# neherlab/pangraph

Measured on AMD Instinct MI355X. Metric: aligned Gbp/s in `pangraph build` (bases handed to the aligner per second, all merges, all self-merge rounds), higher is better.
Workload: dtype u8

## Files before the change

dev/strips_probe.py:

```python
import sys, os, time, faulthandler
ROOT = os.path.dirname(os.path.dirname(os.path.abspath(__file__))); os.chdir(ROOT); sys.path.insert(0, ROOT); sys.path.insert(0, ROOT + '/tests')
faulthandler.dump_traceback_later(240, exit=True)
import numpy as np
import stagebind as sb
from pangraph_amd.mm2ffi import Mm2Lib
from pangraph_amd.synth import random_seq, mutate
gpu = Mm2Lib('pangraph_amd/libpgalign.so')
rng = np.random.default_rng(7)
def job(L, fl, kind):
    t = random_seq(rng, L)
    q = random_seq(rng, L) if kind == "junk" else mutate(rng, t, snp=0.01, indel=0.001)
    if kind == "half": q = np.concatenate([q[:L // 2], random_seq(rng, L // 2)])
    return (sb.nt4(q.tobytes().decode()), sb.nt4(t.tobytes().decode()), 150001, 200, -1, fl)
for L in (10000, 4000, 2048):
    for kind in ("junk", "half", "related"):
        for fl, name in ((0x08, "approx"), (0, "exact")):
            jobs = [job(L, fl, kind)]
            sb.product_extd2(gpu.dll, jobs, 1, 9, 1, 16, 2, 41, 1)
            best = 1e9
            for rep in range(3):
                t0 = time.time(); r = sb.product_extd2(gpu.dll, jobs, 1, 9, 1, 16, 2, 41, 1); best = min(best, time.time() - t0)
            print(f"L={L} {kind:8s} {name:6s}: {best*1e3:7.2f} ms wall; zdropped={r[0]['zdropped']} n_cigar={len(r[0]['cigar'])} score={r[0]['score']}", flush=True)
```

pangraph_amd/csrc/pga_dp.h:

```cpp
#pragma once
#include "pga_common.h"

namespace pga {

struct DpJob {
	uint64_t t_off;
	uint64_t q_off;
	int32_t qlen_full;
	int32_t qs;
	int32_t qlen, tlen;
	int32_t w, zdrop, end_bonus, flag;
	uint8_t q_rev;
	uint8_t seq_rev;
	uint8_t pad[2];
};

struct DpRes {
	int32_t max, max_q, max_t, mqe, mqe_t, mte, mte_q, score;
	int32_t zdropped, reach_end, n_cigar, pad;
	uint64_t cigar_off;
};

#define PGA_JOB_LL 0x8000
#define PGA_LL_MAX_LEN 10240
// ... 5 lines not shown
#include "pga_ksw_shared.h"

namespace pga {

struct LbStop { int32_t on, r_lo, r_hi, tail; };
__host__ __device__ inline int32_t lb_gap(int q, int e, int q2, int e2, int L) { const int a = q + e * L, b = q2 + e2 * L; return a < b ? a : b; }
__host__ __device__ inline LbStop lb_stop_of(int qlen, int tlen, int w, int flag, int q, int e, int q2, int e2, int sc_mch, int sc_mis, int sc_N, int lb_mode)
{
	LbStop S; S.on = 0; S.r_lo = S.r_hi = S.tail = 0;
	if (lb_mode == 1 || (flag & (EZ_APPROX_MAX | PGA_JOB_LL)) || tlen > 64 || tlen < 1 || w < 64 || qlen < w + 2 * tlen) return S;
	if (sc_mch < 0 || sc_mis > sc_mch || sc_N > sc_mch || q < 0 || e < 0 || q2 < 0 || e2 < 0) return S;
	S.on = 1; S.r_lo = 2 * tlen; S.r_hi = w + 30;
	const int qe1 = q + e < q2 + e2 ? q + e : q2 + e2;
	S.tail = tlen > 16 ? sc_mch * tlen - lb_gap(q, e, q2, e2, w + 32 - 2 * tlen) + (sc_mch + qe1) * (2 * tlen - 32) : (int32_t)0x80000000;
	return S;
}
__host__ __device__ inline bool lb_final(const LbStop &S, int r, int tlen, int q, int e, int q2, int e2, int sc_mch, int m)
{
	return S.on && r >= S.r_lo && r <= S.r_hi && sc_mch * tlen - lb_gap(q, e, q2, e2, r + 3 - 2 * tlen) <= m && S.tail <= m;
}

int dp_lb_mode();
void dp_routes_take(int64_t by_class[14], int64_t handed_back[2]);
size_t dp_slab_bytes(int qlen, int tlen, int w);
void dp_run(PkBases d_bases, const std::vector<DpJob> &jobs, const DpParams &P, std::vector<DpRes> &res, PinVec<uint32_t> &cigars, hipStream_t st, Timers *tm = nullptr);

void launch_extd2_fast(int C, unsigned n_waves, const DpJob *jobs, uint32_t n_jobs, PkBases bases, const DpParams &P, uint32_t *counter, uint8_t *slab, size_t slab_bytes,
                       DpRes *res, uint32_t *pool, unsigned long long *cursor, unsigned long long pool_cap, hipStream_t st);

size_t wide_lds_bytes(int r_cap, int seq_cap, bool exact);
void launch_extd2_wide(unsigned n_blocks, int n_threads, int r_cap, int seq_cap, bool exact, const DpJob *jobs, uint32_t n_jobs, PkBases bases, const DpParams &P, uint32_t *counter, uint8_t *slab, size_t slab_bytes,
                       DpRes *res, uint32_t *pool, unsigned long long *cursor, unsigned long long pool_cap, hipStream_t st);

size_t ll_lds_bytes(int t_cap);
size_t ll_multi_scratch_bytes();
int ll_groups(uint32_t n_jobs, int t_max);
void launch_ll_multi(int G, int t_cap, const DpJob *jobs, uint32_t n_jobs, PkBases bases, const DpParams &P, unsigned long long *scratch, DpRes *res, hipStream_t st);
void launch_ll_i16(unsigned n_blocks, int t_cap, const DpJob *jobs, uint32_t n_jobs, PkBases bases, const DpParams &P, uint32_t *counter,
                   unsigned long long *rowkey, size_t rowkey_stride, DpRes *res, hipStream_t st);

size_t band_slab_bytes(int max_diag);
void launch_gapfill_band(unsigned n_waves, const DpJob *jobs, uint32_t n_jobs, PkBases bases, const DpParams &P, uint32_t *counter, uint8_t *slab, size_t slab_bytes,
                         DpRes *res, uint32_t *pool, unsigned long long *cursor, unsigned long long pool_cap, hipStream_t st);

bool strips_eligible(const DpJob &j, const DpParams &P);
size_t strips_slab_bytes(const DpJob &j);
int strips_count(const DpJob &j);
size_t strips_bnd_words(const DpJob &j);
void launch_approx_strips(unsigned n_blocks, const DpJob *jobs, const uint32_t *blk_job, const uint32_t *blk_strip, PkBases bases, const DpParams &P, uint8_t *slab, const uint64_t *slab_off,
                          uint32_t *bnd, const uint64_t *bnd_off, uint32_t *done_ctr, DpRes *res, uint32_t *pool, unsigned long long *cursor, unsigned long long pool_cap, hipStream_t st);

bool wstrips_on();
bool wstrips_eligible(const DpJob &j, const DpParams &P);
int wstrips_count(const DpJob &j);
size_t wstrips_bnd_words(const DpJob &j);
void launch_wstrips(unsigned n_blocks, const DpJob *jobs, const uint32_t *blk_job, const uint32_t *blk_strip, PkBases bases, const DpParams &P, uint8_t *slab, const uint64_t *slab_off,
                    unsigned long long *bnd, const uint64_t *bnd_off, uint32_t *done_ctr, DpRes *res, uint32_t *pool, unsigned long long *cursor, unsigned long long pool_cap, hipStream_t st);
int bstrips_mode();
int bstrips_max_problems();
int bstrips_long_diagonals();
bool bstrips_eligible(const DpJob &j, const DpParams &P);
size_t bstrips_slab_bytes(const DpJob &j);
size_t bstrips_words(const DpJob &j);
uint32_t bstrips_table(const DpJob &j, std::vector<uint32_t> &tab, size_t *words);
void launch_bstrips(unsigned n_blocks, const DpJob *jobs, const uint32_t *blk_job, PkBases bases, const DpParams &P, uint8_t *slab, const uint64_t *slab_off,
                    unsigned long long *bnd, const uint64_t *bnd_off, const uint32_t *tab, const uint64_t *tab_off, DpRes *res, uint32_t *pool, unsigned long long *cursor,
                    unsigned long long pool_cap, hipStream_t st);
bool pipe_eligible(const DpJob &j);
int pipe_mode();
size_t pipe_cig_bytes(int q_cap, int t_cap);
size_t pipe_chunk_bytes();
int pipe_max_chunks();
void launch_ext_pipe(unsigned n_blocks, int q_cap, int t_cap, const DpJob *jobs, uint32_t n_jobs, PkBases bases, const DpParams &P, uint32_t *counter, uint8_t *slab, uint32_t n_chunks,
                     DpRes *res, uint32_t *pool, unsigned long long *cursor, unsigned long long pool_cap, hipStream_t st);
bool lanes_eligible(const DpJob &j, int nt);
size_t lanes_cig_bytes(int q_cap, int t_cap);
size_t lanes_chunk_bytes(int nt);
void launch_extd2_lanes(int nt, unsigned n_blocks, int q_cap, int t_cap, const DpJob *jobs, uint32_t n_jobs, PkBases bases, const DpParams &P, uint32_t *counter, uint8_t *slab, uint32_t n_chunks,
                        DpRes *res, uint32_t *pool, unsigned long long *cursor, unsigned long long pool_cap, hipStream_t st);

}
```

pangraph_amd/csrc/pga_ksw.hip:

```cpp
#include "pga_common.h"
#include "pga_ksw_shared.h"
#include <atomic>
#include <chrono>
#include <mutex>
#include <thread>
#include <array>
#include <cstdio>
#include <cstring>

namespace pga {

#define LDS_T 2048

__global__ __launch_bounds__(64)
void k_extd2(const DpJob *__restrict__ jobs, uint32_t n_jobs, PkBases bases, DpParams P,
             uint32_t *__restrict__ job_counter, uint8_t *__restrict__ slab_all, size_t slab_bytes,
             DpRes *__restrict__ res, uint32_t *__restrict__ cigar_pool, unsigned long long *__restrict__ pool_cursor, unsigned long long pool_cap)
{
	__shared__ int8_t s_rows[7 * LDS_T];
	__shared__ int32_t s_H[LDS_T];
	__shared__ uint32_t s_job;
	const int lane = threadIdx.x;
	uint8_t *slab = slab_all + (size_t)blockIdx.x * slab_bytes;

// ... 578 lines not shown
		lane_need[lane_of_class[c]] = std::max(lane_need[lane_of_class[c]], n_waves * slab_max[c]);
	}
	LaneLease lanes(dev_id, lane_need);
	struct DrainUncollected {
		std::vector<Launch> &L; int dev;
		~DrainUncollected() { for (Launch &X : L) if (X.si >= 0) { (void)sync_stream(X.cs); dp_stream_done(dp_stream_pool(dev), X.si, X.est); X.si = -1; } }
	} drain_uncollected{L, dev_id};
	hipStream_t *lane_stream = lanes.set->stream;
	DBuf<uint8_t> *lane_slab = lanes.set->slab;
	for (int l = 0; l < DP_NLANE; ++l) if (lane_need[l] > lane_slab[l].cap) {
		ArenaScope own(lanes.set->arena);
		g_slab_total -= lane_slab[l].cap; lane_slab[l].alloc(lane_need[l]); g_slab_total += lane_slab[l].cap;
	}
	int lane_si[DP_NLANE] = {-1, -1, -1, -1, -1, -1, -1, -1, -1};
	static const int launch_order[DP_NCLASS] = {13, 12, 9, 11, 7, 6, 5, 4, 3, 10, 2, 8, 1, 0};
	for (int oi = 0; oi < DP_NCLASS; ++oi) {
		const int c = launch_order[oi];
		if (cls[c].empty()) continue;
		std::vector<uint32_t> &ids = cls[c];
		if ((c >= 2 && c != 8) || ids.size() < 100000)
			std::stable_sort(ids.begin(), ids.end(), [&](uint32_t a, uint32_t b) { return (size_t)jobs[a].qlen * jobs[a].tlen > (size_t)jobs[b].qlen * jobs[b].tlen; });
		L.emplace_back();
		Launch &X = L.back();
		X.c = c; X.ids = &ids;
		PinVec<DpJob> &jb = X.jb; jb.resize(ids.size());
		host_parallel(ids.size(), [&](size_t lo, size_t hi) { for (size_t i = lo; i < hi; ++i) jb[i] = jobs[ids[i]]; });
		static const size_t zc_max = getenv("PGA_DP_ZEROCOPY_MAX") ? (size_t)atol(getenv("PGA_DP_ZEROCOPY_MAX")) : 2048;
		X.zc = ids.size() <= zc_max;
		if (X.zc) { X.hr.resize(ids.size()); X.jobs_p = jb.data(); X.res_p = X.hr.data(); }
		else { X.d_jobs.alloc(ids.size()); X.d_r.alloc(ids.size()); X.jobs_p = X.d_jobs.p; X.res_p = X.d_r.p; }
		if (c == 9) { X.d_cnt.alloc(ids.size()); X.cnt_p = X.d_cnt.p; } else X.cnt_p = reinterpret_cast<uint32_t*>(d_cursor.p + 1 + c);
		X.n_waves = waves_of[c];
		uint8_t *slab_p = lane_slab[lane_of_class[c]].p;
		static const bool serial = getenv("PGA_DP_SERIAL") != nullptr;
		hipStream_t cs;
		if (dp_shared_streams()) {
			static const double base_ms[DP_NCLASS] = {1.5, 2.0, 4.0, 6.0, 10.0, 10.0, 10.0, 10.0, 0.5, 12.0, 5.0, 4.0, 2.0, 3.0};
			double est = base_ms[c] * std::max(1.0, (double)ids.size() / (c <= 1 || c == 8 ? 20000.0 : c == 10 || c == 11 || c == 13 ? 512.0 : 64.0));
			DpStreamPool &SP = dp_stream_pool(dev_id);
			int &lsi = lane_si[lane_of_class[c]];
			if (lsi < 0) lsi = dp_stream_pick(SP, est);
			else { std::lock_guard<std::mutex> lk(SP.mu); SP.load[(size_t)lsi] += est; ++SP.pending[(size_t)lsi]; }
			X.si = lsi; X.est = est; cs = SP.st[(size_t)X.si];
		} else cs = lane_stream[serial ? 0 : lane_of_class[c]];
		X.cs = cs;
		if (!X.zc) PGA_HIP(hipMemcpyAsync(X.d_jobs.p, jb.data(), jb.size() * sizeof(DpJob), hipMemcpyHostToDevice, cs));
		if (c == 9) PGA_HIP(hipMemsetAsync(X.d_cnt.p, 0, sizeof(uint32_t) * X.d_cnt.n, cs));
		PGA_HIP(hipEventCreate(&X.e0)); PGA_HIP(hipEventCreate(&X.e1));
		PGA_HIP(hipEventRecord(X.e0, cs));
		if (c == 9) {
			std::vector<uint32_t> &bj = X.h_bj, &bs = X.h_bs; std::vector<uint64_t> &so = X.h_so, &bo = X.h_bo; so.assign(ids.size(), 0); bo.assign(ids.size(), 0);
			uint64_t s_acc = 0, b_acc = 0;
			const bool ws = wstrips_on();
			for (size_t i = 0; i < ids.size(); ++i) {
				const DpJob &j = jobs[ids[i]];
				so[i] = s_acc; s_acc += need[ids[i]];
				bo[i] = b_acc; b_acc += ws ? wstrips_bnd_words(j) : strips_bnd_words(j);
				for (int k2 = 0; k2 < (ws ? wstrips_count(j) : strips_count(j)); ++k2) { bj.push_back((uint32_t)i); bs.push_back((uint32_t)k2); }
			}
			X.d_blk_job.upload(bj, cs); X.d_blk_strip.upload(bs, cs); X.d_slab_off.upload(so, cs); X.d_bnd_off.upload(bo, cs);
			X.d_bnd.alloc(((size_t)b_acc + 1) * (ws ? 2 : 1)); X.d_bnd.zero(cs);
			if (ws) launch_wstrips((unsigned)bj.size(), X.jobs_p, X.d_blk_job.p, X.d_blk_strip.p, d_bases, P, slab_p, X.d_slab_off.p, (unsigned long long*)X.d_bnd.p, X.d_bnd_off.p, X.cnt_p, X.res_p, d_pool.p, d_cursor.p, cig_total, cs);
			else
			launch_approx_strips((unsigned)bj.size(), X.jobs_p, X.d_blk_job.p, X.d_blk_strip.p, d_bases, P, slab_p, X.d_slab_off.p, X.d_bnd.p, X.d_bnd_off.p, X.cnt_p, X.res_p, d_pool.p, d_cursor.p, cig_total, cs);
		} else if (c == 12) {
			std::vector<uint32_t> &bj = X.h_bj, &tab = X.h_tab; std::vector<uint64_t> &so = X.h_so, &bo = X.h_bo, &to = X.h_to; so.assign(ids.size(), 0); bo.assign(ids.size(), 0); to.assign(ids.size(), 0);
			uint64_t s_acc = 0, b_acc = 0;
			for (size_t i = 0; i < ids.size(); ++i) {
				const DpJob &j = jobs[ids[i]];
				so[i] = s_acc; s_acc += need[ids[i]];
				to[i] = tab.size();
				size_t words = 0;
				const uint32_t pool_waves = bstrips_table(j, tab, &words);
				bo[i] = b_acc; b_acc += words;
				for (uint32_t k2 = 0; k2 < pool_waves; ++k2) bj.push_back((uint32_t)i);
			}
			X.d_blk_job.upload(bj, cs); X.d_slab_off.upload(so, cs); X.d_bnd_off.upload(bo, cs); X.d_tab.upload(tab, cs); X.d_tab_off.upload(to, cs);
			X.d_bnd.alloc(((size_t)b_acc + 1) * 2); X.d_bnd.zero(cs);
			X.n_waves = bj.size();
			launch_bstrips((unsigned)bj.size(), X.jobs_p, X.d_blk_job.p, d_bases, P, slab_p, X.d_slab_off.p, (unsigned long long*)X.d_bnd.p, X.d_bnd_off.p, X.d_tab.p, X.d_tab_off.p,
			               X.res_p, d_pool.p, d_cursor.p, cig_total, cs);
		} else if (c == 8) launch_gapfill_band((unsigned)X.n_waves, X.jobs_p, (uint32_t)ids.size(), d_bases, P, X.cnt_p, slab_p, slab_max[c], X.res_p, d_pool.p, d_cursor.p, cig_total, cs);
		else if (c == 6) {
			int t_cap = 16, t_max = 1;
			for (uint32_t id : ids) { t_cap = std::max(t_cap, std::max((jobs[id].tlen + 15) / 16 * 16, (jobs[id].qlen + 15) / 16 * 16)); t_max = std::max(t_max, jobs[id].tlen); }
			const int G = ll_groups((uint32_t)ids.size(), t_max);
			if (G > 1 && ids.size() * ll_multi_scratch_bytes() <= X.n_waves * slab_max[c])
				launch_ll_multi(G, t_cap, X.jobs_p, (uint32_t)ids.size(), d_bases, P, (unsigned long long*)slab_p, X.res_p, cs);
			else
				launch_ll_i16((unsigned)X.n_waves, t_cap, X.jobs_p, (uint32_t)ids.size(), d_bases, P, X.cnt_p, (unsigned long long*)slab_p, slab_max[c] / 8, X.res_p, cs);
		} else if (c <= 1) launch_extd2_fast(c == 0 ? 4 : 8, (unsigned)X.n_waves, X.jobs_p, (uint32_t)ids.size(), d_bases, P, X.cnt_p, slab_p, slab_max[c], X.res_p, d_pool.p, d_cursor.p, cig_total, cs);
		else if (c == 13) {
			int q_cap = 16, t_cap = 16;
			for (uint32_t id : ids) q_cap = std::max(q_cap, jobs[id].qlen), t_cap = std::max(t_cap, jobs[id].tlen);
			launch_ext_pipe((unsigned)X.n_waves, q_cap, t_cap, X.jobs_p, (uint32_t)ids.size(), d_bases, P, X.cnt_p, slab_p, pipe_pool_chunks, X.res_p, d_pool.p, d_cursor.p, cig_total, cs);
		} else if (c == 10 || c == 11) {
			int q_cap = 16, t_cap = 16;
			for (uint32_t id : ids) q_cap = std::max(q_cap, jobs[id].qlen), t_cap = std::max(t_cap, jobs[id].tlen);
			launch_extd2_lanes(c == 11 ? 64 : 256, (unsigned)X.n_waves, q_cap, t_cap, X.jobs_p, (uint32_t)ids.size(), d_bases, P, X.cnt_p, slab_p, lanes_pool_chunks[c - 10], X.res_p, d_pool.p, d_cursor.p, cig_total, cs);
		} else if (c <= 4 || c == 7) {
			int r_cap = 0, seq_cap = 0; bool exact = false;
			for (uint32_t id : ids) { r_cap = std::max(r_cap, wide_ring(jobs[id])); seq_cap = std::max(seq_cap, wide_seqcap(jobs[id])); exact |= !(jobs[id].flag & EZ_APPROX_MAX); }
			if (wide_lds_bytes(r_cap, seq_cap, exact) > WIDE_LDS_MAX) seq_cap = 0;
			static const int c2_seq = getenv("PGA_C2_SEQ") ? atoi(getenv("PGA_C2_SEQ")) : 0;
			if (c == 2 && ids.size() > 1536 && !c2_seq) seq_cap = 0;
			int nt = 256;
			if (c == 4 || c == 7 || ids.size() <= 512) nt = r_cap >= 3000 ? 1024 : r_cap >= 1200 ? 512 : 256;
			if (getenv("PGA_WIDE_NT")) nt = atoi(getenv("PGA_WIDE_NT"));
			else if (c == 3) nt = 512;
			X.nt = nt;
			launch_extd2_wide((unsigned)X.n_waves, nt, r_cap, seq_cap, exact, X.jobs_p, (uint32_t)ids.size(), d_bases, P, X.cnt_p, slab_p, slab_max[c], X.res_p, d_pool.p, d_cursor.p, cig_total, cs);
		} else hipLaunchKernelGGL(k_extd2, dim3((unsigned)X.n_waves), dim3(64), 0, cs, X.jobs_p, (uint32_t)ids.size(), d_bases, P, X.cnt_p, slab_p, slab_max[c],
		                        X.res_p, d_pool.p, d_cursor.p, cig_total);
		PGA_HIP(hipGetLastError());
		PGA_HIP(hipEventRecord(X.e1, cs));
// ... 82 lines not shown
```

pangraph_amd/csrc/pga_ksw_wstrips.hip:

```cpp
#include "pga_common.h"
#include "pga_ksw_shared.h"
#include <cstring>

namespace pga {

#define WS_W 64

__device__ __forceinline__ int ws_sx8(uint32_t v, int sh) { return __builtin_amdgcn_sbfe((int)v, sh, 8); }
__device__ __forceinline__ unsigned long long ws_readlane64(unsigned long long v, int l)
{
	const uint32_t lo = (uint32_t)__builtin_amdgcn_readlane((int)(uint32_t)v, l), hi = (uint32_t)__builtin_amdgcn_readlane((int)(uint32_t)(v >> 32), l);
	return (unsigned long long)hi << 32 | lo;
}

template <bool EXACT>
__device__ __forceinline__ void wstrip_body(const DpJob &J, const uint32_t jl, const uint32_t k, uint8_t *s_win, PkBases bases, const DpParams &P,
               uint8_t *__restrict__ slab_all, const uint64_t *__restrict__ slab_off, unsigned long long *__restrict__ bnd_all, const uint64_t *__restrict__ bnd_off,
               uint32_t *__restrict__ done_ctr, DpRes *__restrict__ res, uint32_t *__restrict__ cigar_pool, unsigned long long *__restrict__ pool_cursor, unsigned long long pool_cap)
{
	const int lane = threadIdx.x;
	const SeqView SV(bases, J);
	const int qlen = J.qlen, tlen = J.tlen;
	const GapCosts G(P);
	const int q = G.q, e = G.e, q2 = G.q2, e2 = G.e2, qe = G.qe, qe2 = G.qe2;
	const int sc_mch = P.sc_mch, sc_mis = P.sc_mis, sc_N = G.sc_N;
	const int qe_h = G.qe_h;
	const int n_strips = (tlen + WS_W - 1) / WS_W;
	const size_t Ld = (size_t)(qlen + tlen);
	const int c0 = (int)k * WS_W, c1 = c0 + WS_W < tlen ? c0 + WS_W : tlen;
	int n_col = qlen < tlen ? qlen : tlen;
	n_col = ((n_col + 15) / 16 + 1) * 16;
	uint8_t *pmat = slab_all + slab_off[jl];
	uint32_t *cig_tmp = (uint32_t*)(pmat + (((size_t)(qlen + tlen - 1) * n_col + 15) & ~(size_t)15));
	unsigned long long *bnd = bnd_all + bnd_off[jl];
	const unsigned long long *bnd_in = k > 0 ? bnd + (size_t)(k - 1) * Ld : nullptr;
	unsigned long long *bnd_out = (int)k + 1 < n_strips ? bnd + (size_t)k * Ld : nullptr;
	int32_t *hen_arr = (int32_t*)(bnd + (size_t)(n_strips > 1 ? n_strips - 1 : 0) * Ld), *hst_arr = hen_arr + Ld;
	const int t = c0 + lane;
	const bool has_col = t < tlen;
	const int tb = SV.target_any(t);
	const int u_first = G.first_row(t);
	int U = u_first, Y = -q - e, Y2 = -q2 - e2, H = KSW_NEG_INF;
	uint32_t PK = ((uint32_t)(-q - e) & 0xffu) | ((uint32_t)(-q - e) & 0xffu) << 8 | ((uint32_t)(-q2 - e2) & 0xffu) << 16;
	int qb = 0;
	const int r_first = c0, r_last = c1 - 1 + qlen - 1;
	const int d_last = c0 + qlen - 2;
	const bool out_strip = bnd_out != nullptr;
	unsigned long long outw = 0;
	uint32_t *s_key = (uint32_t*)s_win;
	unsigned long long *best_arr = (unsigned long long*)(hst_arr + Ld);
	int jq = -lane - 1;
	uint8_t *prow = pmat + (size_t)r_first * n_col;
	{ int st0, en0; diag_range(r_first, qlen, tlen, st0, en0); prow -= st0 / 16 * 16; }
	for (int it0 = 0; r_first + it0 <= r_last; it0 += 64) {
		const int qwin = SV.query(it0 + lane);
		unsigned long long inw = 0;
		{
			const int d = r_first - 1 + it0 + lane;
			if (bnd_in) {
				if (d >= c0 - 1 && d <= d_last)
					for (;;) { inw = __hip_atomic_load(&bnd_in[d], __ATOMIC_RELAXED, __HIP_MEMORY_SCOPE_AGENT); if (inw >> 31 & 1ULL) break; __builtin_amdgcn_s_sleep(2); }
			} else {
				const int rr = d + 1, v1 = G.first_row(rr);
				inw = (unsigned long long)(uint32_t)KSW_NEG_INF << 32 | (((uint32_t)(-q - e) & 0xffu) | ((uint32_t)v1 & 0xffu) << 8 | ((uint32_t)(-q2 - e2) & 0xffu) << 16);
			}
		}
		const int i_end = __builtin_amdgcn_readfirstlane(r_last - (r_first + it0) + 1 < 64 ? r_last - (r_first + it0) + 1 : 64);
		for (int i = 0; i < i_end; ++i) {
			const int r = r_first + it0 + i;
			qb = wave_shr1(qb, __builtin_amdgcn_readlane(qwin, i));
			++jq;
			const bool active = has_col && (unsigned)jq < (unsigned)qlen;
			const uint32_t lw = (uint32_t)wave_shr1((int)PK, __builtin_amdgcn_readlane((int)(uint32_t)inw, i));
			const int xl = ws_sx8(lw, 0), vl = ws_sx8(lw, 8), x2l = ws_sx8(lw, 16);
			int Hl = 0;
			if (EXACT) Hl = wave_shr1(H, __builtin_amdgcn_readlane((int)(uint32_t)(inw >> 32), i));
			int z = tb == qb ? sc_mch : sc_mis;
			z = ((tb | qb) & 4) ? sc_N : z;
			int a = xl + vl, b = Y + U, a2 = x2l + vl, b2 = Y2 + U;
			int d = a > z ? 1 : 0; z = a > z ? a : z;
			d = b > z ? 2 : d; z = b > z ? b : z;
			d = a2 > z ? 3 : d; z = a2 > z ? a2 : z;
			d = b2 > z ? 4 : d; z = b2 > z ? b2 : z;
			z = z < sc_mch ? z : sc_mch;
			const int un = z - vl, vn = z - U;
			int tmp = z - q; a -= tmp; b -= tmp;
			tmp = z - q2; a2 -= tmp; b2 -= tmp;
			d |= a > 0 ? 0x08 : 0; d |= b > 0 ? 0x10 : 0; d |= a2 > 0 ? 0x20 : 0; d |= b2 > 0 ? 0x40 : 0;
			const int xn = (a > 0 ? a : 0) - qe, yn = (b > 0 ? b : 0) - qe, x2n = (a2 > 0 ? a2 : 0) - qe2, y2n = (b2 > 0 ? b2 : 0) - qe2;
			if (active) {
				U = un; Y = yn; Y2 = y2n;
				PK = ((uint32_t)xn & 0xffu) | ((uint32_t)vn & 0xffu) << 8 | ((uint32_t)x2n & 0xffu) << 16;
				prow[(uint32_t)t] = (uint8_t)d;
			}
			if (EXACT) {
				int st0, en0;
				diag_range(r, qlen, tlen, st0, en0);
				uint32_t key = 0;
				if (active) {
					const int en1 = st0 + (en0 - st0) / 4 * 4;
					int h; uint32_t field;
					if (t == en0) { h = r == 0 ? vn - qe_h : en0 > 0 ? Hl + un : H + vn; field = 8u; hen_arr[r] = h; }
					else { h = H + vn; field = 7u - (t < en1 ? (uint32_t)((t - st0) & 3) : 4u); }
					H = h;
					if (t == st0 && r - st0 == qlen - 1) hst_arr[r] = h;
					const int hc = h < -32768 ? -32768 : h > 32767 ? 32767 : h;
					key = ((uint32_t)(hc + 32768) << 16) | field << 12 | (uint32_t)(63 - lane);
				}
				s_key[i * 65 + lane] = key;
			}
			if (out_strip) {
				const uint32_t w63 = (uint32_t)__builtin_amdgcn_readlane((int)PK, 63);
				const bool on63 = (unsigned)(r - (c0 + 63)) < (unsigned)qlen;
				unsigned long long w = on63 ? (0x80000000ULL | w63) : 0ULL;
				if (EXACT) w |= (unsigned long long)(uint32_t)__builtin_amdgcn_readlane(H, 63) << 32;
				if (lane == i) outw = on63 ? w : 0ULL;
			}
			prow += n_col;
			if (r + 2 - qlen > 0 && ((r + 2 - qlen) & 15) == 0) prow -= 16;
		}
		if (out_strip && outw) { __hip_atomic_store(&bnd_out[r_first + it0 + lane], outw, __ATOMIC_RELAXED, __HIP_MEMORY_SCOPE_AGENT); }
		outw = 0;
		if (EXACT) {
			__builtin_amdgcn_fence(__ATOMIC_SEQ_CST, "wavefront");
			if (lane < i_end) {
				uint32_t kb = 0;
#pragma unroll 16
				for (int l = 0; l < 64; ++l) { const uint32_t o = s_key[lane * 65 + l]; kb = o > kb ? o : kb; }
				const unsigned long long comb = (unsigned long long)(kb >> 12) << 20 | (unsigned long long)(4095 - (int)k) << 8 | (unsigned long long)(kb & 255u);
				if (kb) atomicMax(&best_arr[r_first + it0 + lane], comb);
			}
			__builtin_amdgcn_fence(__ATOMIC_SEQ_CST, "wavefront");
		}
	}
	__threadfence();
	uint32_t last = 0;
	if (lane == 0) last = atomicAdd(&done_ctr[jl], 1u);
	last = (uint32_t)__builtin_amdgcn_readfirstlane((int)last);
	if (last + 1 != (uint32_t)n_strips) return;
	__threadfence();
	int bi = tlen - 1, bj = qlen - 1;
	int ez_max = 0, ez_max_t = -1, ez_max_q = -1, ez_mqe = KSW_NEG_INF, ez_mqe_t = -1, ez_mte = KSW_NEG_INF, ez_mte_q = -1, zdropped = 0;
	if (EXACT) {
		const int n_diag = qlen + tlen - 1, zdrop = J.zdrop;
		int sat = 0;
		for (int r0 = 0; r0 < n_diag && !zdropped; r0 += 64) {
			const int r = r0 + lane;
			unsigned long long best = 0; int hen = KSW_NEG_INF, hst = KSW_NEG_INF;
			if (r < n_diag) {
				int st0, en0; diag_range(r, qlen, tlen, st0, en0);
				best = best_arr[r];
				hen = hen_arr[r];
				if (r - st0 == qlen - 1) hst = hst_arr[r];
			}
			const uint32_t h16 = (uint32_t)(best >> 24) & 0xffffu;
			const int mH_l = (int)h16 - 32768, mt_l = (4095 - (int)((best >> 8) & 4095)) * WS_W + (63 - (int)(best & 255));
			const int sat_l = r < n_diag && (h16 == 0 || h16 == 65535u) ? 1 : 0;
			const int lim = n_diag - r0 < 64 ? n_diag - r0 : 64;
			for (int ii = 0; ii < lim; ++ii) {
				const int rr = r0 + ii;
				const int mH = __builtin_amdgcn_readlane(mH_l, ii), mt = __builtin_amdgcn_readlane(mt_l, ii);
				const int he = __builtin_amdgcn_readlane(hen, ii), hs = __builtin_amdgcn_readlane(hst, ii);
				sat |= __builtin_amdgcn_readlane(sat_l, ii);
				int st0, en0; diag_range(rr, qlen, tlen, st0, en0);
				if (en0 == tlen - 1 && he > ez_mte) ez_mte = he, ez_mte_q = rr - en0;
				if (rr - st0 == qlen - 1 && hs > ez_mqe) ez_mqe = hs, ez_mqe_t = st0;
				if (mH > ez_max) ez_max = mH, ez_max_t = mt, ez_max_q = rr - mt;
				else if (mt >= ez_max_t && rr - mt >= ez_max_q) {
					const int tl = mt - ez_max_t, ql = (rr - mt) - ez_max_q, l = tl > ql ? tl - ql : ql - tl;
					if (zdrop >= 0 && ez_max - mH > zdrop + l * e2) { zdropped = 1; break; }
				}
			}
		}
		if (sat) {
			if (lane == 0) { DpRes R; memset(&R, 0, sizeof(R)); R.n_cigar = -9; res[jl] = R; }
			return;
		}
		if (zdropped) bi = ez_max_t, bj = ez_max_q;
	}
	long long guard = 0;
	const int n_cigar = backtrack_windowed<BT_WIN, false>(lane, bi, bj, s_win, cig_tmp, guard, 4000000,
		[&](int r, int &st0, int &en0) { diag_range(r, qlen, tlen, st0, en0); },
		[&](int r, int col) -> uint8_t {
			int st0, en0; diag_range(r, qlen, tlen, st0, en0);
			return st0 <= en0 && col >= st0 && col <= en0 ? pmat[(size_t)r * n_col + (col - st0 / 16 * 16)] : (uint8_t)0;
		});
	__builtin_amdgcn_fence(__ATOMIC_SEQ_CST, "workgroup");
	int score = KSW_NEG_INF;
	if (n_cigar > 0 && !zdropped) {
		int ti = tlen, qj = qlen; score = qe - qe_h;
		for (int c = 0; c < n_cigar; ++c) {
			const uint32_t op = cig_tmp[c] & 0xf; const int len = (int)(cig_tmp[c] >> 4);
			if (op == 0) {
				ti -= len, qj -= len;
				int n_mis = 0, n_amb = 0;
				for (int b = 0; b < len; b += 64) {
					const int l = b + lane;
					bool mis = false, amb = false;
					if (l < len) { const int x = SV.target_any(ti + l), y = SV.query(qj + l); amb = ((x | y) & 4) != 0; mis = !amb && x != y; }
					n_mis += __popcll(__ballot(mis)); n_amb += __popcll(__ballot(amb));
				}
				score += sc_mch * (len - n_mis - n_amb) + sc_mis * n_mis + sc_N * n_amb;
			} else {
				const int g1 = q + len * e, g2 = q2 + len * e2;
				score -= g1 < g2 ? g1 : g2;
				if (op == 1) qj -= len; else ti -= len;
			}
		}
	}
	DpRes R = ez_record(ez_max, ez_max_q, ez_max_t, ez_mqe, ez_mqe_t, ez_mte, ez_mte_q, score, zdropped, 0);
	R.n_cigar = n_cigar, R.pad = qlen + tlen - 1;
	cigar_commit<false, true>(lane, n_cigar, false, cig_tmp, cigar_pool, pool_cursor, pool_cap, R, &res[jl]);
}

__global__ __launch_bounds__(64)
void k_wstrips(const DpJob *__restrict__ jobs, const uint32_t *__restrict__ blk_job, const uint32_t *__restrict__ blk_strip, PkBases bases, DpParams P,
               uint8_t *__restrict__ slab_all, const uint64_t *__restrict__ slab_off, unsigned long long *__restrict__ bnd_all, const uint64_t *__restrict__ bnd_off,
               uint32_t *__restrict__ done_ctr, DpRes *__restrict__ res, uint32_t *__restrict__ cigar_pool, unsigned long long *__restrict__ pool_cursor, unsigned long long pool_cap)
{
	__shared__ __align__(16) uint8_t s_win[64 * 65 * 4];
	const uint32_t jl = blk_job[blockIdx.x], k = blk_strip[blockIdx.x];
	const DpJob J = jobs[jl];
	if (J.flag & EZ_APPROX_MAX) wstrip_body<false>(J, jl, k, s_win, bases, P, slab_all, slab_off, bnd_all, bnd_off, done_ctr, res, cigar_pool, pool_cursor, pool_cap);
	else wstrip_body<true>(J, jl, k, s_win, bases, P, slab_all, slab_off, bnd_all, bnd_off, done_ctr, res, cigar_pool, pool_cursor, pool_cap);
}

bool wstrips_on() { static const bool off = getenv("PGA_OLD_STRIPS") != nullptr; return !off; }
bool wstrips_eligible(const DpJob &j, const DpParams &P)
{
	static const int min_t = getenv("PGA_WSTRIPS_MIN") ? atoi(getenv("PGA_WSTRIPS_MIN")) : 1536;
	static const int min_x = getenv("PGA_WSTRIPS_EXACT_MIN") ? atoi(getenv("PGA_WSTRIPS_EXACT_MIN")) : 2048;
	if (min_t <= 0) return false;
	if (!(j.w >= j.qlen && j.w >= j.tlen && j.qlen >= 256 && j.qlen <= 16384 && j.tlen <= 16384 && P.sc_mch >= 0 && P.sc_mch < 127)) return false;
	if (j.flag == EZ_APPROX_MAX) return j.tlen >= min_t;
	return j.flag == 0 && min_x > 0 && j.tlen >= min_x;
}
int wstrips_count(const DpJob &j) { return (j.tlen + WS_W - 1) / WS_W; }
size_t wstrips_bnd_words(const DpJob &j)
{
	const size_t L = (size_t)(j.qlen + j.tlen), ns = (size_t)wstrips_count(j);
	return (ns > 1 ? ns - 1 : 0) * L + ((j.flag & EZ_APPROX_MAX) ? 0 : (2 * L + 1) / 2 + 1 + L) + 8;
}

void launch_wstrips(unsigned n_blocks, const DpJob *jobs, const uint32_t *blk_job, const uint32_t *blk_strip, PkBases bases, const DpParams &P, uint8_t *slab,
                    const uint64_t *slab_off, unsigned long long *bnd, const uint64_t *bnd_off, uint32_t *done_ctr, DpRes *res, uint32_t *pool, unsigned long long *cursor, unsigned long long pool_cap, hipStream_t st)
{
	hipLaunchKernelGGL(k_wstrips, dim3(n_blocks), dim3(64), 0, st, jobs, blk_job, blk_strip, bases, P, slab, slab_off, bnd, bnd_off, done_ctr, res, pool, cursor, pool_cap);
}

}
```

Measured before the change: 7.860.

## Add concurrent z-drop evaluator block to stop exact wide strips early

For exact (non-approx) wide-strip jobs, an extra evaluator block is launched per job. It watches per-64-diagonal completion counters, runs the z-drop scan incrementally and publishes a stop word. Strip blocks poll that word and stop filling the DP matrix once z-drop is detected, so diagonals past the drop point are no longer computed. The cost is extra atomics and fences per diagonal block, an additional block per job that spins while it waits, and a possible deadlock if the evaluator block is not co-resident with the strips (a poll limit guards this).

```diff
diff --git a/dev/strips_probe.py b/dev/strips_probe.py
--- a/dev/strips_probe.py
+++ b/dev/strips_probe.py
@@ -5,19 +5,20 @@
 import stagebind as sb
 from pangraph_amd.mm2ffi import Mm2Lib
 from pangraph_amd.synth import random_seq, mutate
-gpu = Mm2Lib('pangraph_amd/libpgalign.so')
+gpu = Mm2Lib(os.environ.get('PGA_LIB') or 'pangraph_amd/libpgalign.so')
 rng = np.random.default_rng(7)
 def job(L, fl, kind):
     t = random_seq(rng, L)
     q = random_seq(rng, L) if kind == "junk" else mutate(rng, t, snp=0.01, indel=0.001)
     if kind == "half": q = np.concatenate([q[:L // 2], random_seq(rng, L // 2)])
+    if kind == "early": q = np.concatenate([q[:500], random_seq(rng, L - 500)])
     return (sb.nt4(q.tobytes().decode()), sb.nt4(t.tobytes().decode()), 150001, 200, -1, fl)
 for L in (10000, 4000, 2048):
-    for kind in ("junk", "half", "related"):
+    for kind in ("junk", "early", "half", "related"):
         for fl, name in ((0x08, "approx"), (0, "exact")):
             jobs = [job(L, fl, kind)]
             sb.product_extd2(gpu.dll, jobs, 1, 9, 1, 16, 2, 41, 1)
             best = 1e9
-            for rep in range(3):
+            for rep in range(5):
                 t0 = time.time(); r = sb.product_extd2(gpu.dll, jobs, 1, 9, 1, 16, 2, 41, 1); best = min(best, time.time() - t0)
             print(f"L={L} {kind:8s} {name:6s}: {best*1e3:7.2f} ms wall; zdropped={r[0]['zdropped']} n_cigar={len(r[0]['cigar'])} score={r[0]['score']}", flush=True)
diff --git a/dev/wstrips_stop_dist.py b/dev/wstrips_stop_dist.py
--- /dev/null
+++ b/dev/wstrips_stop_dist.py
@@ -0,0 +1,20 @@
+import sys
+import numpy as np
+rows = [[int(x) for x in ln.split()[3::2]] for ln in sys.stdin if ln.startswith("[wstrips prof]")]
+if not rows:
+    sys.exit("no [wstrips prof] lines")
+a = np.array(rows, dtype=np.int64)
+ql, tl, nd, re, zd = a.T
+def cells_upto(ql, tl, r):
+    r = np.minimum(r, ql + tl - 1); lo, hi = np.minimum(ql, tl), np.maximum(ql, tl)
+    tri = np.minimum(r, lo); c = tri * (tri + 1) // 2
+    mid = np.clip(r - lo, 0, hi - lo); c = c + mid * lo
+    tail = np.clip(r - hi, 0, lo - 1); c = c + tail * lo - tail * (tail + 1) // 2
+    return c
+allc = ql * tl
+used = cells_upto(ql, tl, np.where(zd == 1, re + 1, nd))
+frac = np.where(zd == 1, (re + 1) / nd, 1.0)
+q = np.percentile(frac[zd == 1], [25, 50, 75]) if zd.any() else [1, 1, 1]
+print(f"exact problems {len(a)}; zdropped {int(zd.sum())} ({zd.mean():.1%}); r*/n_diag of the z-dropped: quartiles {q[0]:.3f} {q[1]:.3f} {q[2]:.3f}")
+print(f"cells: all {allc.sum():.4g}, on diagonals <= r* {used.sum():.4g}, beyond r* {allc.sum() - used.sum():.4g} ({1 - used.sum() / allc.sum():.1%} of all)")
+print(f"diagonals: all {nd.sum()}, up to r* {int(np.where(zd == 1, re + 1, nd).sum())}; median n_diag {int(np.median(nd))}, largest {int(nd.max())}")
diff --git a/pangraph_amd/csrc/pga_dp.h b/pangraph_amd/csrc/pga_dp.h
--- a/pangraph_amd/csrc/pga_dp.h
+++ b/pangraph_amd/csrc/pga_dp.h
@@ -81,10 +81,12 @@
 
 bool wstrips_on();
 bool wstrips_eligible(const DpJob &j, const DpParams &P);
+bool wstrips_stop();
 int wstrips_count(const DpJob &j);
+int wstrips_blocks(const DpJob &j, bool stop);
 size_t wstrips_bnd_words(const DpJob &j);
 void launch_wstrips(unsigned n_blocks, const DpJob *jobs, const uint32_t *blk_job, const uint32_t *blk_strip, PkBases bases, const DpParams &P, uint8_t *slab, const uint64_t *slab_off,
-                    unsigned long long *bnd, const uint64_t *bnd_off, uint32_t *done_ctr, DpRes *res, uint32_t *pool, unsigned long long *cursor, unsigned long long pool_cap, hipStream_t st);
+                    unsigned long long *bnd, const uint64_t *bnd_off, uint32_t *done_ctr, DpRes *res, uint32_t *pool, unsigned long long *cursor, unsigned long long pool_cap, bool stop, hipStream_t st);
 int bstrips_mode();
 int bstrips_max_problems();
 int bstrips_long_diagonals();
diff --git a/pangraph_amd/csrc/pga_ksw.hip b/pangraph_amd/csrc/pga_ksw.hip
--- a/pangraph_amd/csrc/pga_ksw.hip
+++ b/pangraph_amd/csrc/pga_ksw.hip
@@ -654,15 +654,16 @@
 			std::vector<uint32_t> &bj = X.h_bj, &bs = X.h_bs; std::vector<uint64_t> &so = X.h_so, &bo = X.h_bo; so.assign(ids.size(), 0); bo.assign(ids.size(), 0);
 			uint64_t s_acc = 0, b_acc = 0;
 			const bool ws = wstrips_on();
+			const bool ws_stop = ws && wstrips_stop();
 			for (size_t i = 0; i < ids.size(); ++i) {
 				const DpJob &j = jobs[ids[i]];
 				so[i] = s_acc; s_acc += need[ids[i]];
 				bo[i] = b_acc; b_acc += ws ? wstrips_bnd_words(j) : strips_bnd_words(j);
-				for (int k2 = 0; k2 < (ws ? wstrips_count(j) : strips_count(j)); ++k2) { bj.push_back((uint32_t)i); bs.push_back((uint32_t)k2); }
+				for (int k2 = 0; k2 < (ws ? wstrips_blocks(j, ws_stop) : strips_count(j)); ++k2) { bj.push_back((uint32_t)i); bs.push_back((uint32_t)k2); }
 			}
 			X.d_blk_job.upload(bj, cs); X.d_blk_strip.upload(bs, cs); X.d_slab_off.upload(so, cs); X.d_bnd_off.upload(bo, cs);
 			X.d_bnd.alloc(((size_t)b_acc + 1) * (ws ? 2 : 1)); X.d_bnd.zero(cs);
-			if (ws) launch_wstrips((unsigned)bj.size(), X.jobs_p, X.d_blk_job.p, X.d_blk_strip.p, d_bases, P, slab_p, X.d_slab_off.p, (unsigned long long*)X.d_bnd.p, X.d_bnd_off.p, X.cnt_p, X.res_p, d_pool.p, d_cursor.p, cig_total, cs);
+			if (ws) launch_wstrips((unsigned)bj.size(), X.jobs_p, X.d_blk_job.p, X.d_blk_strip.p, d_bases, P, slab_p, X.d_slab_off.p, (unsigned long long*)X.d_bnd.p, X.d_bnd_off.p, X.cnt_p, X.res_p, d_pool.p, d_cursor.p, cig_total, ws_stop, cs);
 			else
 			launch_approx_strips((unsigned)bj.size(), X.jobs_p, X.d_blk_job.p, X.d_blk_strip.p, d_bases, P, slab_p, X.d_slab_off.p, X.d_bnd.p, X.d_bnd_off.p, X.cnt_p, X.res_p, d_pool.p, d_cursor.p, cig_total, cs);
 		} else if (c == 12) {
diff --git a/pangraph_amd/csrc/pga_ksw_wstrips.hip b/pangraph_amd/csrc/pga_ksw_wstrips.hip
--- a/pangraph_amd/csrc/pga_ksw_wstrips.hip
+++ b/pangraph_amd/csrc/pga_ksw_wstrips.hip
@@ -13,10 +13,78 @@
 	return (unsigned long long)hi << 32 | lo;
 }
 
+struct WsPtrs { uint8_t *pmat; uint32_t *cig_tmp, *stop_w, *done_blk; unsigned long long *bnd, *best_arr; int32_t *hen_arr, *hst_arr; int n_strips, n_col; size_t Ld; };
+__device__ __forceinline__ WsPtrs ws_ptrs(const DpJob &J, const uint32_t jl, uint8_t *__restrict__ slab_all, const uint64_t *__restrict__ slab_off,
+                                          unsigned long long *__restrict__ bnd_all, const uint64_t *__restrict__ bnd_off)
+{
+	WsPtrs W;
+	const int qlen = J.qlen, tlen = J.tlen;
+	W.n_strips = (tlen + WS_W - 1) / WS_W;
+	W.Ld = (size_t)(qlen + tlen);
+	int n_col = qlen < tlen ? qlen : tlen;
+	W.n_col = ((n_col + 15) / 16 + 1) * 16;
+	W.pmat = slab_all + slab_off[jl];
+	W.cig_tmp = (uint32_t*)(W.pmat + (((size_t)(qlen + tlen - 1) * W.n_col + 15) & ~(size_t)15));
+	W.bnd = bnd_all + bnd_off[jl];
+	W.hen_arr = (int32_t*)(W.bnd + (size_t)(W.n_strips > 1 ? W.n_strips - 1 : 0) * W.Ld), W.hst_arr = W.hen_arr + W.Ld;
+	W.best_arr = (unsigned long long*)(W.hst_arr + W.Ld);
+	W.stop_w = (uint32_t*)(W.best_arr + W.Ld), W.done_blk = W.stop_w + 2;
+	return W;
+}
+__host__ __device__ inline int ws_need(int b, int n_strips, int qlen)
+{
+	const int m = (qlen + 62) >> 6;
+	const int lo = b - m > 0 ? b - m : 0, hi = b < n_strips - 2 ? b : n_strips - 2;
+	return (hi >= lo ? hi - lo + 1 : 0) + (b >= n_strips - 1 ? 1 : 0);
+}
+
+struct WsEz { int max, max_t, max_q, mqe, mqe_t, mte, mte_q, zdropped, sat, r_end; };
+__device__ __forceinline__ WsEz ws_ez_init(int n_diag)
+{
+	WsEz S;
+	S.max = 0, S.max_t = -1, S.max_q = -1, S.mqe = KSW_NEG_INF, S.mqe_t = -1, S.mte = KSW_NEG_INF, S.mte_q = -1, S.zdropped = 0, S.sat = 0, S.r_end = n_diag;
+	return S;
+}
+__device__ __forceinline__ bool ws_eval_block(WsEz &S, const int r0, const int lane, const int qlen, const int tlen, const int zdrop, const int e2, const WsPtrs &W)
+{
+	const int n_diag = qlen + tlen - 1, r = r0 + lane;
+	unsigned long long best = 0; int hen = KSW_NEG_INF, hst = KSW_NEG_INF;
+	if (r < n_diag) {
+		int st0, en0; diag_range(r, qlen, tlen, st0, en0);
+		best = __hip_atomic_load(&W.best_arr[r], __ATOMIC_RELAXED, __HIP_MEMORY_SCOPE_AGENT);
+		hen = __hip_atomic_load(&W.hen_arr[r], __ATOMIC_RELAXED, __HIP_MEMORY_SCOPE_AGENT);
+		if (r - st0 == qlen - 1) hst = __hip_atomic_load(&W.hst_arr[r], __ATOMIC_RELAXED, __HIP_MEMORY_SCOPE_AGENT);
+	}
+	const uint32_t h16 = (uint32_t)(best >> 24) & 0xffffu;
+	const int mH_l = (int)h16 - 32768, mt_l = (4095 - (int)((best >> 8) & 4095)) * WS_W + (63 - (int)(best & 255));
+	const int sat_l = r < n_diag && (h16 == 0 || h16 == 65535u) ? 1 : 0;
+	const int lim = n_diag - r0 < 64 ? n_diag - r0 : 64;
+	for (int ii = 0; ii < lim; ++ii) {
+		const int rr = r0 + ii;
+		const int mH = __builtin_amdgcn_readlane(mH_l, ii), mt = __builtin_amdgcn_readlane(mt_l, ii);
+		const int he = __builtin_amdgcn_readlane(hen, ii), hs = __builtin_amdgcn_readlane(hst, ii);
+		S.sat |= __builtin_amdgcn_readlane(sat_l, ii);
+		int st0, en0; diag_range(rr, qlen, tlen, st0, en0);
+		if (en0 == tlen - 1 && he > S.mte) S.mte = he, S.mte_q = rr - en0;
+		if (rr - st0 == qlen - 1 && hs > S.mqe) S.mqe = hs, S.mqe_t = st0;
+		if (mH > S.max) S.max = mH, S.max_t = mt, S.max_q = rr - mt;
+		else if (mt >= S.max_t && rr - mt >= S.max_q) {
+			const int tl = mt - S.max_t, ql = (rr - mt) - S.max_q, l = tl > ql ? tl - ql : ql - tl;
+			if (zdrop >= 0 && S.max - mH > zdrop + l * e2) { S.zdropped = 1, S.r_end = rr; return true; }
+		}
+	}
+	return false;
+}
+
+template <bool EXACT>
+__device__ __forceinline__ void wstrip_finish(const DpJob &J, const uint32_t jl, const int lane, const WsEz &S, const WsPtrs &W, uint8_t *s_win, PkBases bases, const DpParams &P,
+               DpRes *__restrict__ res, uint32_t *__restrict__ cigar_pool, unsigned long long *__restrict__ pool_cursor, unsigned long long pool_cap);
+
 template <bool EXACT>
 __device__ __forceinline__ void wstrip_body(const DpJob &J, const uint32_t jl, const uint32_t k, uint8_t *s_win, PkBases bases, const DpParams &P,
                uint8_t *__restrict__ slab_all, const uint64_t *__restrict__ slab_off, unsigned long long *__restrict__ bnd_all, const uint64_t *__restrict__ bnd_off,
-               uint32_t *__restrict__ done_ctr, DpRes *__restrict__ res, uint32_t *__restrict__ cigar_pool, unsigned long long *__restrict__ pool_cursor, unsigned long long pool_cap)
+               uint32_t *__restrict__ done_ctr, DpRes *__restrict__ res, uint32_t *__restrict__ cigar_pool, unsigned long long *__restrict__ pool_cursor, unsigned long long pool_cap,
+               const bool stop_on)
 {
 	const int lane = threadIdx.x;
 	const SeqView SV(bases, J);
@@ -25,17 +93,16 @@
 	const int q = G.q, e = G.e, q2 = G.q2, e2 = G.e2, qe = G.qe, qe2 = G.qe2;
 	const int sc_mch = P.sc_mch, sc_mis = P.sc_mis, sc_N = G.sc_N;
 	const int qe_h = G.qe_h;
-	const int n_strips = (tlen + WS_W - 1) / WS_W;
-	const size_t Ld = (size_t)(qlen + tlen);
+	const WsPtrs W = ws_ptrs(J, jl, slab_all, slab_off, bnd_all, bnd_off);
+	const int n_strips = W.n_strips, n_col = W.n_col;
+	const size_t Ld = W.Ld;
 	const int c0 = (int)k * WS_W, c1 = c0 + WS_W < tlen ? c0 + WS_W : tlen;
-	int n_col = qlen < tlen ? qlen : tlen;
-	n_col = ((n_col + 15) / 16 + 1) * 16;
-	uint8_t *pmat = slab_all + slab_off[jl];
-	uint32_t *cig_tmp = (uint32_t*)(pmat + (((size_t)(qlen + tlen - 1) * n_col + 15) & ~(size_t)15));
-	unsigned long long *bnd = bnd_all + bnd_off[jl];
+	uint8_t *pmat = W.pmat;
+	unsigned long long *bnd = W.bnd;
 	const unsigned long long *bnd_in = k > 0 ? bnd + (size_t)(k - 1) * Ld : nullptr;
 	unsigned long long *bnd_out = (int)k + 1 < n_strips ? bnd + (size_t)k * Ld : nullptr;
-	int32_t *hen_arr = (int32_t*)(bnd + (size_t)(n_strips > 1 ? n_strips - 1 : 0) * Ld), *hst_arr = hen_arr + Ld;
+	int32_t *hen_arr = W.hen_arr, *hst_arr = W.hst_arr;
+	const bool stopping = EXACT && stop_on;
 	const int t = c0 + lane;
 	const bool has_col = t < tlen;
 	const int tb = SV.target_any(t);
@@ -48,23 +115,31 @@
 	const bool out_strip = bnd_out != nullptr;
 	unsigned long long outw = 0;
 	uint32_t *s_key = (uint32_t*)s_win;
-	unsigned long long *best_arr = (unsigned long long*)(hst_arr + Ld);
+	unsigned long long *best_arr = W.best_arr;
 	int jq = -lane - 1;
 	uint8_t *prow = pmat + (size_t)r_first * n_col;
 	{ int st0, en0; diag_range(r_first, qlen, tlen, st0, en0); prow -= st0 / 16 * 16; }
 	for (int it0 = 0; r_first + it0 <= r_last; it0 += 64) {
+		uint32_t stop_seen = 0;
+		if (stopping) stop_seen = __hip_atomic_load((const uint32_t*)(best_arr + Ld), __ATOMIC_RELAXED, __HIP_MEMORY_SCOPE_AGENT);
 		const int qwin = SV.query(it0 + lane);
 		unsigned long long inw = 0;
 		{
 			const int d = r_first - 1 + it0 + lane;
 			if (bnd_in) {
 				if (d >= c0 - 1 && d <= d_last)
-					for (;;) { inw = __hip_atomic_load(&bnd_in[d], __ATOMIC_RELAXED, __HIP_MEMORY_SCOPE_AGENT); if (inw >> 31 & 1ULL) break; __builtin_amdgcn_s_sleep(2); }
+					for (;;) {
+						inw = __hip_atomic_load(&bnd_in[d], __ATOMIC_RELAXED, __HIP_MEMORY_SCOPE_AGENT);
+						if (inw >> 31 & 1ULL) break;
+						if (stopping && __hip_atomic_load((const uint32_t*)(best_arr + Ld), __ATOMIC_RELAXED, __HIP_MEMORY_SCOPE_AGENT) != 0u) { stop_seen = 1; break; }
+						__builtin_amdgcn_s_sleep(2);
+					}
 			} else {
 				const int rr = d + 1, v1 = G.first_row(rr);
 				inw = (unsigned long long)(uint32_t)KSW_NEG_INF << 32 | (((uint32_t)(-q - e) & 0xffu) | ((uint32_t)v1 & 0xffu) << 8 | ((uint32_t)(-q2 - e2) & 0xffu) << 16);
 			}
 		}
+		if (stopping && __ballot(stop_seen != 0u) != 0ULL) break;
 		const int i_end = __builtin_amdgcn_readfirstlane(r_last - (r_first + it0) + 1 < 64 ? r_last - (r_first + it0) + 1 : 64);
 		for (int i = 0; i < i_end; ++i) {
 			const int r = r_first + it0 + i;
@@ -131,52 +206,46 @@
 				if (kb) atomicMax(&best_arr[r_first + it0 + lane], comb);
 			}
 			__builtin_amdgcn_fence(__ATOMIC_SEQ_CST, "wavefront");
-		}
-	}
+			if (stopping) {
+				__threadfence();
+				if (lane == 0) (void)__hip_atomic_fetch_add((uint32_t*)(best_arr + Ld) + 2 + ((r_first + it0) >> 6), 1u, __ATOMIC_RELAXED, __HIP_MEMORY_SCOPE_AGENT);
+			}
+		}
+	}
+	if (stopping) return;
 	__threadfence();
 	uint32_t last = 0;
 	if (lane == 0) last = atomicAdd(&done_ctr[jl], 1u);
 	last = (uint32_t)__builtin_amdgcn_readfirstlane((int)last);
 	if (last + 1 != (uint32_t)n_strips) return;
 	__threadfence();
+	WsEz S = ws_ez_init(qlen + tlen - 1);
+	if (EXACT) for (int r0 = 0; r0 < qlen + tlen - 1; r0 += 64) if (ws_eval_block(S, r0, lane, qlen, tlen, J.zdrop, e2, W)) break;
+	wstrip_finish<EXACT>(J, jl, lane, S, W, s_win, bases, P, res, cigar_pool, pool_cursor, pool_cap);
+}
+
+template <bool EXACT>
+__device__ __forceinline__ void wstrip_finish(const DpJob &J, const uint32_t jl, const int lane, const WsEz &S, const WsPtrs &W, uint8_t *s_win, PkBases bases, const DpParams &P,
+               DpRes *__restrict__ res, uint32_t *__restrict__ cigar_pool, unsigned long long *__restrict__ pool_cursor, unsigned long long pool_cap)
+{
+	const SeqView SV(bases, J);
+	const int qlen = J.qlen, tlen = J.tlen, n_col = W.n_col;
+	const GapCosts G(P);
+	const int q = G.q, e = G.e, q2 = G.q2, e2 = G.e2, qe = G.qe, qe_h = G.qe_h;
+	const int sc_mch = P.sc_mch, sc_mis = P.sc_mis, sc_N = G.sc_N;
+	const uint8_t *pmat = W.pmat;
+	uint32_t *cig_tmp = W.cig_tmp;
+	const int zdropped = S.zdropped;
 	int bi = tlen - 1, bj = qlen - 1;
-	int ez_max = 0, ez_max_t = -1, ez_max_q = -1, ez_mqe = KSW_NEG_INF, ez_mqe_t = -1, ez_mte = KSW_NEG_INF, ez_mte_q = -1, zdropped = 0;
 	if (EXACT) {
-		const int n_diag = qlen + tlen - 1, zdrop = J.zdrop;
-		int sat = 0;
-		for (int r0 = 0; r0 < n_diag && !zdropped; r0 += 64) {
-			const int r = r0 + lane;
-			unsigned long long best = 0; int hen = KSW_NEG_INF, hst = KSW_NEG_INF;
-			if (r < n_diag) {
-				int st0, en0; diag_range(r, qlen, tlen, st0, en0);
-				best = best_arr[r];
-				hen = hen_arr[r];
-				if (r - st0 == qlen - 1) hst = hst_arr[r];
-			}
-			const uint32_t h16 = (uint32_t)(best >> 24) & 0xffffu;
-			const int mH_l = (int)h16 - 32768, mt_l = (4095 - (int)((best >> 8) & 4095)) * WS_W + (63 - (int)(best & 255));
-			const int sat_l = r < n_diag && (h16 == 0 || h16 == 65535u) ? 1 : 0;
-			const int lim = n_diag - r0 < 64 ? n_diag - r0 : 64;
-			for (int ii = 0; ii < lim; ++ii) {
-				const int rr = r0 + ii;
-				const int mH = __builtin_amdgcn_readlane(mH_l, ii), mt = __builtin_amdgcn_readlane(mt_l, ii);
-				const int he = __builtin_amdgcn_readlane(hen, ii), hs = __builtin_amdgcn_readlane(hst, ii);
-				sat |= __builtin_amdgcn_readlane(sat_l, ii);
-				int st0, en0; diag_range(rr, qlen, tlen, st0, en0);
-				if (en0 == tlen - 1 && he > ez_mte) ez_mte = he, ez_mte_q = rr - en0;
-				if (rr - st0 == qlen - 1 && hs > ez_mqe) ez_mqe = hs, ez_mqe_t = st0;
-				if (mH > ez_max) ez_max = mH, ez_max_t = mt, ez_max_q = rr - mt;
-				else if (mt >= ez_max_t && rr - mt >= ez_max_q) {
-					const int tl = mt - ez_max_t, ql = (rr - mt) - ez_max_q, l = tl > ql ? tl - ql : ql - tl;
-					if (zdrop >= 0 && ez_max - mH > zdrop + l * e2) { zdropped = 1; break; }
-				}
-			}
-		}
-		if (sat) {
+#ifdef PGA_WS_PROF
+		if (lane == 0) printf("[wstrips prof] qlen %d tlen %d n_diag %d r_end %d zdropped %d\n", qlen, tlen, qlen + tlen - 1, S.r_end, zdropped);
+#endif
+		if (S.sat) {
 			if (lane == 0) { DpRes R; memset(&R, 0, sizeof(R)); R.n_cigar = -9; res[jl] = R; }
 			return;
 		}
-		if (zdropped) bi = ez_max_t, bj = ez_max_q;
+		if (zdropped) bi = S.max_t, bj = S.max_q;
 	}
 	long long guard = 0;
 	const int n_cigar = backtrack_windowed<BT_WIN, false>(lane, bi, bj, s_win, cig_tmp, guard, 4000000,
@@ -208,21 +277,45 @@
 			}
 		}
 	}
-	DpRes R = ez_record(ez_max, ez_max_q, ez_max_t, ez_mqe, ez_mqe_t, ez_mte, ez_mte_q, score, zdropped, 0);
+	DpRes R = ez_record(S.max, S.max_q, S.max_t, S.mqe, S.mqe_t, S.mte, S.mte_q, score, zdropped, 0);
 	R.n_cigar = n_cigar, R.pad = qlen + tlen - 1;
 	cigar_commit<false, true>(lane, n_cigar, false, cig_tmp, cigar_pool, pool_cursor, pool_cap, R, &res[jl]);
+}
+
+__device__ __forceinline__ void wstrip_evaluate(const DpJob &J, const uint32_t jl, uint8_t *s_win, PkBases bases, const DpParams &P,
+               uint8_t *__restrict__ slab_all, const uint64_t *__restrict__ slab_off, unsigned long long *__restrict__ bnd_all, const uint64_t *__restrict__ bnd_off,
+               DpRes *__restrict__ res, uint32_t *__restrict__ cigar_pool, unsigned long long *__restrict__ pool_cursor, unsigned long long pool_cap)
+{
+	const int lane = threadIdx.x;
+	const int qlen = J.qlen, tlen = J.tlen, n_diag = qlen + tlen - 1, nblk = (n_diag + 63) / 64;
+	const GapCosts G(P);
+	const WsPtrs W = ws_ptrs(J, jl, slab_all, slab_off, bnd_all, bnd_off);
+	WsEz S = ws_ez_init(n_diag);
+	bool halt = false;
+	for (int b = 0; b < nblk && !halt; ++b) {
+		const uint32_t need = (uint32_t)ws_need(b, W.n_strips, qlen);
+		long long polls = 0;
+		while (__hip_atomic_load(&W.done_blk[b], __ATOMIC_ACQUIRE, __HIP_MEMORY_SCOPE_AGENT) < need) { if (++polls > 20000000LL) { S.sat = 1; break; } __builtin_amdgcn_s_sleep(8); }
+		if (S.sat) break;
+		__threadfence();
+		halt = ws_eval_block(S, b * 64, lane, qlen, tlen, J.zdrop, G.e2, W) || S.sat;
+	}
+	if (lane == 0) __hip_atomic_store(W.stop_w, (uint32_t)S.r_end + 1u, __ATOMIC_RELEASE, __HIP_MEMORY_SCOPE_AGENT);
+	wstrip_finish<true>(J, jl, lane, S, W, s_win, bases, P, res, cigar_pool, pool_cursor, pool_cap);
 }
 
 __global__ __launch_bounds__(64)
 void k_wstrips(const DpJob *__restrict__ jobs, const uint32_t *__restrict__ blk_job, const uint32_t *__restrict__ blk_strip, PkBases bases, DpParams P,
                uint8_t *__restrict__ slab_all, const uint64_t *__restrict__ slab_off, unsigned long long *__restrict__ bnd_all, const uint64_t *__restrict__ bnd_off,
-               uint32_t *__restrict__ done_ctr, DpRes *__restrict__ res, uint32_t *__restrict__ cigar_pool, unsigned long long *__restrict__ pool_cursor, unsigned long long pool_cap)
+               uint32_t *__restrict__ done_ctr, DpRes *__restrict__ res, uint32_t *__restrict__ cigar_pool, unsigned long long *__restrict__ pool_cursor, unsigned long long pool_cap,
+               int stop_on)
 {
 	__shared__ __align__(16) uint8_t s_win[64 * 65 * 4];
 	const uint32_t jl = blk_job[blockIdx.x], k = blk_strip[blockIdx.x];
 	const DpJob J = jobs[jl];
-	if (J.flag & EZ_APPROX_MAX) wstrip_body<false>(J, jl, k, s_win, bases, P, slab_all, slab_off, bnd_all, bnd_off, done_ctr, res, cigar_pool, pool_cursor, pool_cap);
-	else wstrip_body<true>(J, jl, k, s_win, bases, P, slab_all, slab_off, bnd_all, bnd_off, done_ctr, res, cigar_pool, pool_cursor, pool_cap);
+	if (J.flag & EZ_APPROX_MAX) wstrip_body<false>(J, jl, k, s_win, bases, P, slab_all, slab_off, bnd_all, bnd_off, done_ctr, res, cigar_pool, pool_cursor, pool_cap, false);
+	else if ((int)k == (J.tlen + WS_W - 1) / WS_W) wstrip_evaluate(J, jl, s_win, bases, P, slab_all, slab_off, bnd_all, bnd_off, res, cigar_pool, pool_cursor, pool_cap);
+	else wstrip_body<true>(J, jl, k, s_win, bases, P, slab_all, slab_off, bnd_all, bnd_off, done_ctr, res, cigar_pool, pool_cursor, pool_cap, stop_on != 0);
 }
 
 bool wstrips_on() { static const bool off = getenv("PGA_OLD_STRIPS") != nullptr; return !off; }
@@ -235,17 +328,19 @@
 	if (j.flag == EZ_APPROX_MAX) return j.tlen >= min_t;
 	return j.flag == 0 && min_x > 0 && j.tlen >= min_x;
 }
+bool wstrips_stop() { const char *e = getenv("PGA_WSTRIPS_STOP"); return !e || (strcmp(e, "0") && strcmp(e, "off")); }
 int wstrips_count(const DpJob &j) { return (j.tlen + WS_W - 1) / WS_W; }
+int wstrips_blocks(const DpJob &j, bool stop) { return wstrips_count(j) + (stop && !(j.flag & EZ_APPROX_MAX) ? 1 : 0); }
 size_t wstrips_bnd_words(const DpJob &j)
 {
-	const size_t L = (size_t)(j.qlen + j.tlen), ns = (size_t)wstrips_count(j);
-	return (ns > 1 ? ns - 1 : 0) * L + ((j.flag & EZ_APPROX_MAX) ? 0 : (2 * L + 1) / 2 + 1 + L) + 8;
+	const size_t L = (size_t)(j.qlen + j.tlen), ns = (size_t)wstrips_count(j), nblk = (L + 62) / 64;
+	return (ns > 1 ? ns - 1 : 0) * L + ((j.flag & EZ_APPROX_MAX) ? 0 : (2 * L + 1) / 2 + 1 + L + 1 + (nblk + 1) / 2) + 8;
 }
 
 void launch_wstrips(unsigned n_blocks, const DpJob *jobs, const uint32_t *blk_job, const uint32_t *blk_strip, PkBases bases, const DpParams &P, uint8_t *slab,
-                    const uint64_t *slab_off, unsigned long long *bnd, const uint64_t *bnd_off, uint32_t *done_ctr, DpRes *res, uint32_t *pool, unsigned long long *cursor, unsigned long long pool_cap, hipStream_t st)
-{
-	hipLaunchKernelGGL(k_wstrips, dim3(n_blocks), dim3(64), 0, st, jobs, blk_job, blk_strip, bases, P, slab, slab_off, bnd, bnd_off, done_ctr, res, pool, cursor, pool_cap);
-}
-
-}
+                    const uint64_t *slab_off, unsigned long long *bnd, const uint64_t *bnd_off, uint32_t *done_ctr, DpRes *res, uint32_t *pool, unsigned long long *cursor, unsigned long long pool_cap, bool stop, hipStream_t st)
+{
+	hipLaunchKernelGGL(k_wstrips, dim3(n_blocks), dim3(64), 0, st, jobs, blk_job, blk_strip, bases, P, slab, slab_off, bnd, bnd_off, done_ctr, res, pool, cursor, pool_cap, stop ? 1 : 0);
+}
+
+}
```

Measured after the change: 6.983. 0.888x the previous value.
